# vrenkens/tfkaldi

Hardware: AMD Instinct MI355X
Metric: acoustic frames/sec (train step) (higher is better)
Workload: dtype f32 emulated (3xbf16 planes, 6 products, f32 accumulate)

## Files before the change

tfkaldi_amd/csrc/gemm_bf16.hip:

```cpp
#include "gemm_bf16.h"
#include "x3_layout.h"

#include <math.h>
#include <stdlib.h>
#include <string.h>

#include <type_traits>

namespace tfk {
namespace {

typedef __bf16 bf16x8 __attribute__((ext_vector_type(8)));
typedef __bf16 bf16x4 __attribute__((ext_vector_type(4)));
typedef float f32x16 __attribute__((ext_vector_type(16)));
typedef uint32_t u32x4 __attribute__((ext_vector_type(4)));
typedef int i32x4 __attribute__((ext_vector_type(4)));

constexpr int BK = 64;
constexpr int kOOB = (int)0x80000000;
constexpr int NUM_XCD = 8;

__device__ __forceinline__ void tile_of_seq(int tiles_m, int tiles_n, int group_rows, int seq, int& tm, int& tn) {
  const int per_group = group_rows * tiles_n;
  const int grp = seq / per_group;
// ... 324 lines not shown
  template <bool GUARD>
  __device__ __forceinline__ void issue(int j, unsigned image, int k0, int wave) const {
    const int off = (!GUARD || k0 + kidx[j] < k_lim) ? voff[j] : kOOB;
    const unsigned dst = image + (unsigned)(wave * 64 + j * NTH) * 16u;
    const int soff = k0 * kstride;
    asm volatile("s_mov_b32 m0, %0\n\ts_nop 0\n\tbuffer_load_dwordx4 %1, %2, %3 offen lds"
                 :
                 : "s"(dst), "v"(off), "s"(rsrc), "s"(soff)
                 : "memory");
  }
};

template <bool KC, int EXT, int NF>
struct Frag3 {
  int off[2];
  __device__ __forceinline__ void init(int lane, int frag0) {
#pragma unroll
    for (int v = 0; v < 2; ++v) off[v] = KC ? x3::kc_lane_off(lane, frag0, v) : x3::ks_lane_off<EXT>(lane, frag0, v);
  }
  __device__ __forceinline__ Frag3 at(int bytes) const {
    Frag3 r;
    r.off[0] = off[0] + bytes;
    r.off[1] = off[1] + bytes;
    return r;
  }
  __device__ __forceinline__ bf16x8 read(const char* img, int f, int ks, int pl) const {
    if constexpr (KC) {
      return *reinterpret_cast<const bf16x8*>(img + off[ks] + x3::kc_imm(f, pl));
    } else {
      typedef __attribute__((address_space(3))) bf16x4 lds_bf16x4;
      const int X = 3 * f + pl;
      const char* q = img + off[X & 1];
      const bf16x4 lo = __builtin_amdgcn_ds_read_tr16_b64_v4bf16((lds_bf16x4*)(q + x3::ks_imm<EXT>(X, ks, 0)));
      const bf16x4 hi = __builtin_amdgcn_ds_read_tr16_b64_v4bf16((lds_bf16x4*)(q + x3::ks_imm<EXT>(X, ks, 1)));
      return __builtin_shufflevector(lo, hi, 0, 1, 2, 3, 4, 5, 6, 7);
    }
  }
};

template <bool KC, int EXT, int NF16>
struct Frag3M {
  int off[KC ? 1 : 4];
  __device__ __forceinline__ void init(int lane, int frag0) {
    if constexpr (KC) {
      off[0] = x3::kc16_lane_off(lane, frag0);
    } else {
#pragma unroll
      for (int v = 0; v < 4; ++v) off[v] = x3::ks16_lane_off<EXT>(lane, frag0, v & 1, v >> 1);
    }
  }
  __device__ __forceinline__ Frag3M at(int bytes) const {
    Frag3M r;
#pragma unroll
    for (int v = 0; v < (KC ? 1 : 4); ++v) r.off[v] = off[v] + bytes;
    return r;
  }
  __device__ __forceinline__ bf16x8 read(const char* img, int f, int pl) const {
    if constexpr (KC) {
      return *reinterpret_cast<const bf16x8*>(img + off[0] + x3::kc16_imm(f, pl));
    } else {
      typedef __attribute__((address_space(3))) bf16x4 lds_bf16x4;
      const int X = 3 * (f >> 1) + pl;
      const char* q = img + off[(X & 1) + 2 * (f & 1)];
      const bf16x4 lo = __builtin_amdgcn_ds_read_tr16_b64_v4bf16((lds_bf16x4*)(q + x3::ks16_imm<EXT>(X, 0)));
      const bf16x4 hi = __builtin_amdgcn_ds_read_tr16_b64_v4bf16((lds_bf16x4*)(q + x3::ks16_imm<EXT>(X, 1)));
      return __builtin_shufflevector(lo, hi, 0, 1, 2, 3, 4, 5, 6, 7);
    }
  }
};

#ifndef TFKB_ABL
#define TFKB_ABL 0
#endif

#ifndef TFKB_TL
#define TFKB_TL(ev, ti)
#endif

#define TFKB_WAIT_BARRIER(n) \
  asm volatile("s_waitcnt vmcnt(%0)\n\ts_waitcnt lgkmcnt(0)\n\ts_barrier" : : "n"(n) : "memory")

constexpr int kSplitFlagWords = 4096;
constexpr int kSplitXccWord = 2048;
template <bool A_KC, bool B_KC, int EPI, int WAVES_M, int WAVES_N, int FM, int FN, int NS, int BKT = 64, int SCHED = 0,
          int NPL = 1, int KSPLIT = 1, int LOADERS = 0, bool LIST = false, bool CBUF = false>
__device__ __forceinline__ void dma_tile(const GemmArgsB& p, int tiles_m, int tiles_n, int group_rows, int bid, char* smem,
                                         int seq0 = 0, int ntiles = 1) {
  static_assert(LOADERS == 0 || (NPL == 3 && LOADERS == WAVES_M * WAVES_N), "loader waves: one per multiplying wave, x3 only");
  static_assert(!LIST || (NPL == 3 && KSPLIT == 1 && LOADERS == 0), "tile lists: the unsplit fp32-emulating contraction, no loader waves");
  constexpr int NTH = WAVES_M * WAVES_N * 64;
  constexpr int BM = WAVES_M * FM * 32, BN = WAVES_N * FN * 32;
  typedef typename std::conditional<NPL == 3, DmaOperand3<A_KC, BM, NTH>, DmaOperand<A_KC, BM, NTH, BKT>>::type OA;
  typedef typename std::conditional<NPL == 3, DmaOperand3<B_KC, BN, NTH>, DmaOperand<B_KC, BN, NTH, BKT>>::type OB;
  constexpr int A_BYTES = BM * BKT * 2, B_BYTES = BN * BKT * 2, STAGE = NPL * (A_BYTES + B_BYTES);
  constexpr int NPA = OA::NP, NPB = OB::NP, NP = OA::NP + OB::NP;
  constexpr int KSPT = BKT / 16;
  static_assert(KSPT == 4 || KSPT == 2, "ring slot of 64 or 32 k");
  static_assert(NS >= 3 && (NS - 2) * NP + (NPL == 3 ? NP / 2 : 0) <= 63, "ring depth / vmcnt range");
  static_assert(FM * FN >= 2 || NPL == 3, "two independent accumulator chains per wave");
  static_assert(NPL == 1 || (NPL == 3 && SCHED == 0), "planes");
  static_assert(KSPLIT == 1 || (KSPLIT == 2 && NPL == 3), "split-K: the fp32-emulating contraction only");

  const int tid = threadIdx.x;
  const int lane = tid & 63;
  const int i = lane & 31, h = lane >> 5;
  const int wave = __builtin_amdgcn_readfirstlane(tid >> 6);
  const int wm = wave / WAVES_N, wn = wave % WAVES_N;
  int tm, tn;
  const int khalf = KSPLIT == 2 ? (bid / NUM_XCD) & 1 : 0;
  const int tile_bid = KSPLIT == 2 ? (bid / NUM_XCD >> 1) * NUM_XCD + bid % NUM_XCD : bid;
  if constexpr (LIST) tile_of_seq(tiles_m, tiles_n, group_rows, seq0, tm, tn);
  else tile_of_block(tiles_m, tiles_n, group_rows, tile_bid, tm, tn);
  int m0 = tm * BM, n0 = tn * BN;
  unsigned my_xcc = 0;
  if constexpr (KSPLIT == 2) {
    if (p.splitk_local) {
      asm volatile("s_getreg_b32 %0, hwreg(HW_REG_XCC_ID, 0, 4)" : "=s"(my_xcc));
      if (tid == 0)
        __hip_atomic_store(reinterpret_cast<unsigned*>(p.splitk_ws) + kSplitXccWord + 2 * (tm * tiles_n + tn) + khalf, my_xcc + 1,
                           __ATOMIC_RELAXED, __HIP_MEMORY_SCOPE_AGENT);
    }
  }

  const int K8 = (p.K + 7) & ~7;
  const int nk_all = (p.K + BKT - 1) / BKT;
  const int h0 = KSPLIT == 2 ? max(1, (nk_all + 1) / 2 - p.splitk_skew) : nk_all;
  const int kbase = khalf ? h0 : 0;
  const int nk = KSPLIT == 2 ? (khalf ? nk_all - h0 : h0) : nk_all;
  const int k_end = (kbase + nk) * BKT;
  const unsigned lds0 = __builtin_amdgcn_readfirstlane((unsigned)(unsigned long long)smem);
  OA la;
  OB lb;
  const int a_klim = min(A_KC ? K8 : p.K, k_end), b_klim = min(B_KC ? K8 : p.K, k_end);
  const int nk_full = min(a_klim, b_klim) / BKT - kbase;
  if constexpr (LOADERS > 0) {
    if (wave >= WAVES_M * WAVES_N) {
      const int lwave = wave - WAVES_M * WAVES_N;
      la.init(p.A, p.lda, A_KC ? p.M : p.K, m0, A_KC ? p.M : ((p.M + 7) & ~7), a_klim, tid - NTH);
      lb.init(p.B, p.ldb, B_KC ? p.N : p.K, n0, B_KC ? p.N : ((p.N + 7) & ~7), b_klim, tid - NTH);
      auto tile = [&](auto guard, int slot, int kt) {
        if (TFKB_ABL & 2) return;
#pragma unroll
        for (int j = 0; j < NPA; ++j)
          la.template issue<decltype(guard)::value>(j, lds0 + (unsigned)(slot * STAGE), (kt + kbase) * BKT, lwave);
#pragma unroll
        for (int j = 0; j < NPB; ++j)
          lb.template issue<decltype(guard)::value>(j, lds0 + (unsigned)(slot * STAGE + NPL * A_BYTES), (kt + kbase) * BKT, lwave);
      };
#pragma unroll
      for (int t = 0; t < NS - 1; ++t) tile(std::true_type(), t, t);
      TFKB_WAIT_BARRIER((NS - 2) * NP);
      int ws = NS - 1;
      const int n_fast = max(0, min(nk, nk_full - (NS - 1)));
#pragma unroll 1
      for (int kt = 0; kt < nk; ++kt) {
        if (kt < n_fast) tile(std::false_type(), ws, kt + NS - 1);
        else tile(std::true_type(), ws, kt + NS - 1);
        TFKB_WAIT_BARRIER((NS - 2) * NP);
        ws = ws + 1 == NS ? 0 : ws + 1;
      }
      TFKB_WAIT_BARRIER(0);
      return;
    }
  }
  auto init_loaders = [&]() {
    if constexpr (LOADERS == 0) {
// ... 42 lines not shown
        lb.issue(j - NPA, lds0 + (unsigned)(slot * STAGE + A_BYTES), (kt + kbase) * BKT, wave);
    }
  };
  auto piece = [&](int j, int slot, int kt) { piece_g(std::true_type(), j, slot, kt); };
  constexpr int NPH = NPL == 3 ? NP / 2 : 0;
  auto prologue = [&]() {
#pragma unroll
    for (int t = 0; t < NS - 1; ++t)
#pragma unroll
      for (int j = 0; j < NP; ++j) piece(j, t, t);
#pragma unroll
    for (int j = 0; j < NPH; ++j) piece(j, NS - 1, NS - 1);
    TFKB_WAIT_BARRIER((NS - 2) * NP + NPH);
  };

  bf16x8 fa[2][NPL][FM], fb[2][NPL][FN];
  auto read_frags = [&](int buf, const char* st, int ks) {
    if (TFKB_ABL & 4) return;
#pragma unroll
    for (int pl = 0; pl < NPL; ++pl) {
      if constexpr (NPL == 3) {
#pragma unroll
        for (int a = 0; a < FM; ++a) fa[buf][pl][a] = qa.read(st, a, ks, pl);
#pragma unroll
        for (int b = 0; b < FN; ++b) fb[buf][pl][b] = qb.read(st + NPL * A_BYTES, b, ks, pl);
      } else {
#pragma unroll
        for (int a = 0; a < FM; ++a) fa[buf][pl][a] = qa.read(st, a, ks);
#pragma unroll
        for (int b = 0; b < FN; ++b) fb[buf][pl][b] = qb.read(st + A_BYTES, b, ks);
      }
    }
  };
  if (TFKB_ABL & 4) {
#pragma unroll
    for (int q = 0; q < 2; ++q) {
#pragma unroll
      for (int pl = 0; pl < NPL; ++pl) {
#pragma unroll
        for (int a = 0; a < FM; ++a)
#pragma unroll
          for (int e = 0; e < 8; ++e) fa[q][pl][a][e] = (__bf16)(float)(lane + e + pl);
#pragma unroll
        for (int b = 0; b < FN; ++b)
#pragma unroll
          for (int e = 0; e < 8; ++e) fb[q][pl][b][e] = (__bf16)(float)(lane - e - pl);
      }
    }
  }
  auto mfma_step = [&](int cur) {
    if (TFKB_ABL & 1) {
#pragma unroll
      for (int pl = 0; pl < NPL; ++pl) {
#pragma unroll
        for (int a = 0; a < FM; ++a) asm volatile("" : : "v"(fa[cur][pl][a]));
#pragma unroll
        for (int b = 0; b < FN; ++b) asm volatile("" : : "v"(fb[cur][pl][b]));
      }
    } else if constexpr (NPL == 1) {
#pragma unroll
      for (int a = 0; a < FM; ++a)
#pragma unroll
        for (int b = 0; b < FN; ++b)
          acc[a][b] = __builtin_amdgcn_mfma_f32_32x32x16_bf16(fa[cur][0][a], fb[cur][0][b], acc[a][b], 0, 0, 0);
    } else {
      constexpr int PA[6] = {2, 1, 0, 1, 0, 0}, PB[6] = {0, 1, 2, 0, 1, 0};
#pragma unroll
      for (int c = 0; c < 5; ++c)
#pragma unroll
        for (int a = 0; a < FM; ++a)
#pragma unroll
          for (int b = 0; b < FN; ++b)
            acc2[a][b] = __builtin_amdgcn_mfma_f32_32x32x16_bf16(fa[cur][PA[c]][a], fb[cur][PB[c]][b], acc2[a][b], 0, 0, 0);
#pragma unroll
      for (int a = 0; a < FM; ++a)
#pragma unroll
        for (int b = 0; b < FN; ++b)
          acc[a][b] = __builtin_amdgcn_mfma_f32_32x32x16_bf16(fa[cur][0][a], fb[cur][0][b], acc[a][b], 0, 0, 0);
    }
  };
  constexpr bool CHAIN = LIST && NPL == 3 && TFK_X3_M16 == 0 && SCHED == 0;
  const int nlist = LIST ? ntiles : 1;
  float* const red = reinterpret_cast<float*>(smem + (LIST ? NS * STAGE : 0));
  bool primed = false;
  int rs = 0, ws = NS - 1;
#pragma unroll 1
  for (int ti = 0; ti < nlist; ++ti) {
    TFKB_TL(0, ti);
    if (!primed) {
      if (ti > 0) {
        tile_of_seq(tiles_m, tiles_n, group_rows, seq0 + ti, tm, tn);
        m0 = tm * BM;
        n0 = tn * BN;
        init_loaders();
      }
      prologue();
      rs = 0;
      ws = NS - 1;
    }
    zero_acc();
    const bool chain_next = CHAIN && nk >= NS && ti + 1 < nlist;
    const int tm_out = tm, m0_out = m0, n0_out = n0;
    if constexpr (SCHED == 2) {
      static_assert(WAVES_M * WAVES_N == 8, "two waves per SIMD");
      const int group = wave >> 2;
      bf16x8 wa[KSPT][FM], wb[KSPT][FN];
      if (group == 1) {
        __builtin_amdgcn_sched_barrier(0);
        asm volatile("s_barrier" : : : "memory");
        __builtin_amdgcn_sched_barrier(0);
      }
#pragma unroll 1
      for (int kt = 0; kt < nk; ++kt) {
        const char* st = smem + rs * STAGE;
#pragma unroll
        for (int ks = 0; ks < KSPT; ++ks) {
#pragma unroll
          for (int a = 0; a < FM; ++a) wa[ks][a] = qa.read(st, a, ks);
#pragma unroll
          for (int b = 0; b < FN; ++b) wb[ks][b] = qb.read(st + A_BYTES, b, ks);
        }
#pragma unroll
        for (int j = 0; j < NP; ++j) piece(j, ws, kt + NS - 1);
        __builtin_amdgcn_sched_barrier(0);
        TFKB_WAIT_BARRIER((NS - 2) * NP);
        __builtin_amdgcn_sched_barrier(0);
#pragma unroll
        for (int ks = 0; ks < KSPT; ++ks)
#pragma unroll
          for (int a = 0; a < FM; ++a)
#pragma unroll
            for (int b = 0; b < FN; ++b)
              acc[a][b] = __builtin_amdgcn_mfma_f32_32x32x16_bf16(wa[ks][a], wb[ks][b], acc[a][b], 0, 0, 0);
        rs = rs + 1 == NS ? 0 : rs + 1;
        ws = ws + 1 == NS ? 0 : ws + 1;
        __builtin_amdgcn_sched_barrier(0);
        asm volatile("s_barrier" : : : "memory");
        __builtin_amdgcn_sched_barrier(0);
      }
      if (group == 0) {
        __builtin_amdgcn_sched_barrier(0);
        asm volatile("s_barrier" : : : "memory");
        __builtin_amdgcn_sched_barrier(0);
      }
    } else if constexpr (NPL == 3 && TFK_X3_M16 != 0) {
      static_assert(KSPT == 2, "fp32-emulating contraction: 32 k per ring slot");
      constexpr int FM16 = 2 * FM, FN16 = 2 * FN;
      typedef float f32x4 __attribute__((ext_vector_type(4)));
      Frag3M<A_KC, BM, FM16> ma;
      Frag3M<B_KC, BN, FN16> mb;
      ma.init(lane, wm * FM16);
      mb.init(lane, wn * FN16);
      f32x4 c1[FM16][FN16], c2[FM16][FN16];
#pragma unroll
      for (int a = 0; a < FM16; ++a)
#pragma unroll
        for (int b = 0; b < FN16; ++b) {
          c1[a][b] = f32x4{0.f, 0.f, 0.f, 0.f};
          c2[a][b] = f32x4{0.f, 0.f, 0.f, 0.f};
        }
      bf16x8 ga[3][FM16], gb[3][FN16], gb0n[FN16];
      auto rd_a = [&](const decltype(ma)& r, int pl) {
#pragma unroll
        for (int a = 0; a < FM16; ++a) ga[pl][a] = r.read(smem, a, pl);
      };
      auto rd_b = [&](const decltype(mb)& r, int pl, bf16x8 (&dst)[FN16]) {
#pragma unroll
        for (int b = 0; b < FN16; ++b) dst[b] = r.read(smem, b, pl);
      };
      auto mm = [&](int pa, int pb) {
#pragma unroll
        for (int a = 0; a < FM16; ++a)
#pragma unroll
          for (int b = 0; b < FN16; ++b) {
            if (pa + pb == 0) c1[a][b] = __builtin_amdgcn_mfma_f32_16x16x32_bf16(ga[0][a], gb[0][b], c1[a][b], 0, 0, 0);
            else c2[a][b] = __builtin_amdgcn_mfma_f32_16x16x32_bf16(ga[pa][a], gb[pb][b], c2[a][b], 0, 0, 0);
          }
        __builtin_amdgcn_sched_barrier(0);
      };
      auto pieces = [&](auto guard, int part, int j0, int j1, int slot, int tile) {
#pragma unroll
        for (int j = j0 + part * (j1 - j0) / 3; j < j0 + (part + 1) * (j1 - j0) / 3; ++j) piece_g(guard, j, slot, tile);
      };
      {
        const auto r0a = ma.at(0);
        const auto r0b = mb.at(NPL * A_BYTES);
        rd_a(r0a, 0);
        rd_b(r0b, 0, gb[0]);
        rd_b(r0b, 1, gb[1]);
        rd_b(r0b, 2, gb[2]);
      }
      const int n_fast = max(0, min(nk, nk_full - NS));
      auto iteration = [&](auto guard, int kt) {
        const auto ra = ma.at(rs * STAGE);
        rd_a(ra, 1);
        pieces(guard, 0, NPH, NP, ws, kt + NS - 1);
        mm(0, 0);
        rd_a(ra, 2);
        pieces(guard, 1, NPH, NP, ws, kt + NS - 1);
        mm(0, 1);
        pieces(guard, 2, NPH, NP, ws, kt + NS - 1);
        mm(0, 2);
        TFKB_WAIT_BARRIER((NS - 2) * NP);
        rs = rs + 1 == NS ? 0 : rs + 1;
        ws = ws + 1 == NS ? 0 : ws + 1;
        const bool fetch = kt + 1 < nk;
        const auto na = ma.at(rs * STAGE);
        const auto nb = mb.at(rs * STAGE + NPL * A_BYTES);
        if (fetch) {
          rd_a(na, 0);
          rd_b(nb, 0, gb0n);
        }
        pieces(guard, 0, 0, NPH, ws, kt + NS);
        mm(1, 0);
        if (fetch) rd_b(nb, 2, gb[2]);
        pieces(guard, 1, 0, NPH, ws, kt + NS);
        mm(1, 1);
        if (fetch) rd_b(nb, 1, gb[1]);
        pieces(guard, 2, 0, NPH, ws, kt + NS);
        mm(2, 0);
        if (fetch) {
#pragma unroll
          for (int b = 0; b < FN16; ++b) gb[0][b] = gb0n[b];
        }
      };
#pragma unroll 1
      for (int kt = 0; kt < n_fast; ++kt) iteration(std::false_type(), kt);
#pragma unroll 1
      for (int kt = n_fast; kt < nk; ++kt) iteration(std::true_type(), kt);
      {
        const int src = (16 * h + (i & 15)) * 4;
#pragma unroll
        for (int a = 0; a < FM; ++a)
#pragma unroll
          for (int b = 0; b < FN; ++b)
#pragma unroll
            for (int r = 0; r < 16; ++r) {
              const int addr = src + (((r >> 2) & 1) ? 128 : 0);
              const f32x4& t0 = c1[2 * a + (r >> 3)][2 * b], &u0 = c2[2 * a + (r >> 3)][2 * b];
              const f32x4& t1 = c1[2 * a + (r >> 3)][2 * b + 1], &u1 = c2[2 * a + (r >> 3)][2 * b + 1];
              const float v0 = __builtin_bit_cast(float, __builtin_amdgcn_ds_bpermute(addr, __builtin_bit_cast(int, t0[r & 3] + u0[r & 3])));
              const float v1 = __builtin_bit_cast(float, __builtin_amdgcn_ds_bpermute(addr, __builtin_bit_cast(int, t1[r & 3] + u1[r & 3])));
              acc[a][b][r] = (i & 16) ? v1 : v0;
            }
      }
    } else if constexpr (NPL == 3) {
      static_assert(KSPT == 2, "fp32-emulating contraction: 32 k per ring slot");
      constexpr int PA[6] = {2, 1, 0, 1, 0, 0}, PB[6] = {0, 1, 2, 0, 1, 0};
      auto step3 = [&](auto guard, int cur, bool fetch, const decltype(qa)& ra, const decltype(qb)& rb, int nks, int j0, int j1,
                       int slot, int tile) {
#pragma unroll
        for (int c = 0; c < 6; ++c) {
          if (c < 3 && fetch && !(TFKB_ABL & 4)) {
#pragma unroll
            for (int a = 0; a < FM; ++a) fa[cur ^ 1][PA[c]][a] = ra.read(smem, a, nks, PA[c]);
#pragma unroll
            for (int b = 0; b < FN; ++b) fb[cur ^ 1][PB[c]][b] = rb.read(smem, b, nks, PB[c]);
          }
#pragma unroll
          for (int j = j0 + c * (j1 - j0) / 6; j < j0 + (c + 1) * (j1 - j0) / 6; ++j) piece_g(guard, j, slot, tile);
          if (TFKB_ABL & 1) {
#pragma unroll
            for (int a = 0; a < FM; ++a) asm volatile("" : : "v"(fa[cur][PA[c]][a]));
#pragma unroll
            for (int b = 0; b < FN; ++b) asm volatile("" : : "v"(fb[cur][PB[c]][b]));
          } else {
#pragma unroll
            for (int a = 0; a < FM; ++a)
#pragma unroll
              for (int b = 0; b < FN; ++b) {
                if (c < 5)
                  acc2[a][b] = __builtin_amdgcn_mfma_f32_32x32x16_bf16(fa[cur][PA[c]][a], fb[cur][PB[c]][b], acc2[a][b], 0, 0, 0);
                else
                  acc[a][b] = __builtin_amdgcn_mfma_f32_32x32x16_bf16(fa[cur][PA[c]][a], fb[cur][PB[c]][b], acc[a][b], 0, 0, 0);
              }
          }
          __builtin_amdgcn_sched_barrier(0);
        }
      };
      if (!primed) read_frags(0, smem, 0);
      const int n_fast = max(0, min(nk, nk_full - NS));
      auto iteration = [&](auto guard, int t1, int t2, bool fetch, bool switch_tile) {
        const auto ra = qa.at(rs * STAGE);
        const auto rb = qb.at(rs * STAGE + NPL * A_BYTES);
        step3(guard, 0, true, ra, rb, 1, NPH, NP, ws, t1);
        TFKB_WAIT_BARRIER((NS - 2) * NP);
        rs = rs + 1 == NS ? 0 : rs + 1;
        ws = ws + 1 == NS ? 0 : ws + 1;
        if constexpr (CHAIN) {
          if (switch_tile) {
            tile_of_seq(tiles_m, tiles_n, group_rows, seq0 + ti + 1, tm, tn);
            m0 = tm * BM;
            n0 = tn * BN;
            init_loaders();
          }
        }
        const auto na = qa.at(rs * STAGE);
        const auto nb = qb.at(rs * STAGE + NPL * A_BYTES);
        step3(guard, 1, fetch, na, nb, 0, 0, NPH, ws, t2);
      };
      const int n_own = chain_next ? nk - NS : nk;
      TFKB_TL(1, ti);
#pragma unroll 1
      for (int kt = 0; kt < n_fast; ++kt) iteration(std::false_type(), kt + NS - 1, kt + NS, kt + 1 < nk, false);
#pragma unroll 1
      for (int kt = n_fast; kt < n_own; ++kt) iteration(std::true_type(), kt + NS - 1, kt + NS, kt + 1 < nk, false);
      if constexpr (CHAIN) {
        if (chain_next) {
          iteration(std::true_type(), nk - 1, 0, true, true);
#pragma unroll 1
          for (int t = 0; t < NS - 1; ++t) iteration(std::true_type(), t, t + 1, true, false);
        }
      }
      TFKB_TL(2, ti);
    } else {
    read_frags(0, smem, 0);
#pragma unroll 1
    for (int kt = 0; kt < nk; ++kt) {
      const char* st = smem + rs * STAGE;
#pragma unroll
      for (int ks = 0; ks < KSPT - 1; ++ks) {
        const int cur = ks & 1;
        read_frags(cur ^ 1, st, ks + 1);
#pragma unroll
        for (int j = ks * NP / (KSPT - 1); j < (ks + 1) * NP / (KSPT - 1); ++j) piece(j, ws, kt + NS - 1);
        mfma_step(cur);
        __builtin_amdgcn_sched_barrier(0);
      }
      TFKB_WAIT_BARRIER((NS - 2) * NP);
      rs = rs + 1 == NS ? 0 : rs + 1;
      ws = ws + 1 == NS ? 0 : ws + 1;
      if (kt + 1 < nk) read_frags(0, smem + rs * STAGE, 0);
      mfma_step((KSPT - 1) & 1);
      __builtin_amdgcn_sched_barrier(0);
    }
    }
    if (!chain_next) TFKB_WAIT_BARRIER(0);
    if constexpr (NPL == 3) {
#pragma unroll
      for (int a = 0; a < FM; ++a)
#pragma unroll
        for (int b = 0; b < FN; ++b)
#pragma unroll
          for (int r = 0; r < 16; ++r) acc[a][b][r] += acc2[a][b][r];
    }
    if constexpr (KSPLIT == 2) {
      typedef float f32x4 __attribute__((ext_vector_type(4)));
      unsigned* flags = reinterpret_cast<unsigned*>(p.splitk_ws);
      const int tile = tm * tiles_n + tn;
      constexpr int kSys = 1 | (1 << 4);
      __amdgpu_buffer_rsrc_t part = __builtin_amdgcn_make_buffer_rsrc(
          (void*)(p.splitk_ws + kSplitFlagWords + (size_t)tile * (BM * BN)), 0, BM * BN * 4, 0x00020000);
      unsigned* sh = reinterpret_cast<unsigned*>(smem);
      if (tid == 0) {
        sh[0] = __hip_atomic_fetch_add(&flags[2 * tile], 1u, __ATOMIC_RELAXED, __HIP_MEMORY_SCOPE_AGENT);
        sh[1] = p.splitk_local ? __hip_atomic_load(&flags[kSplitXccWord + 2 * tile + (khalf ^ 1)], __ATOMIC_RELAXED, __HIP_MEMORY_SCOPE_AGENT)
                               : 0u;
      }
      __syncthreads();
      const bool first = sh[0] == 0;
      if (first) {
        const bool same_xcd = p.splitk_local && sh[1] == my_xcc + 1;
        if (same_xcd) {
#pragma unroll
          for (int a = 0; a < FM; ++a)
#pragma unroll
            for (int b = 0; b < FN; ++b)
#pragma unroll
              for (int q = 0; q < 4; ++q)
                __builtin_amdgcn_raw_buffer_store_b128(
                    __builtin_bit_cast(u32x4, f32x4{acc[a][b][4 * q], acc[a][b][4 * q + 1], acc[a][b][4 * q + 2], acc[a][b][4 * q + 3]}),
                    part, ((((wave * FM + a) * FN + b) * 4 + q) * 64 + lane) * 16, 0, 0);
        } else {
#pragma unroll
          for (int a = 0; a < FM; ++a)
#pragma unroll
            for (int b = 0; b < FN; ++b)
#pragma unroll
              for (int q = 0; q < 4; ++q)
                __builtin_amdgcn_raw_buffer_store_b128(
                    __builtin_bit_cast(u32x4, f32x4{acc[a][b][4 * q], acc[a][b][4 * q + 1], acc[a][b][4 * q + 2], acc[a][b][4 * q + 3]}),
                    part, ((((wave * FM + a) * FN + b) * 4 + q) * 64 + lane) * 16, 0, kSys);
        }
        asm volatile("s_waitcnt vmcnt(0)" : : : "memory");
        __syncthreads();
        if (tid == 0) __hip_atomic_store(&flags[2 * tile + 1], 1u, __ATOMIC_RELAXED, __HIP_MEMORY_SCOPE_AGENT);
        return;
      }
      if (tid == 0) {
        int spin = 0;
        for (; spin < (1 << 23) && __hip_atomic_load(&flags[2 * tile + 1], __ATOMIC_RELAXED, __HIP_MEMORY_SCOPE_AGENT) == 0; ++spin)
          __builtin_amdgcn_s_sleep(2);
        if (spin == (1 << 23) && p.err) __hip_atomic_store(p.err, 1u, __ATOMIC_RELAXED, __HIP_MEMORY_SCOPE_SYSTEM);
        __hip_atomic_store(&flags[2 * tile], 0u, __ATOMIC_RELAXED, __HIP_MEMORY_SCOPE_AGENT);
        __hip_atomic_store(&flags[2 * tile + 1], 0u, __ATOMIC_RELAXED, __HIP_MEMORY_SCOPE_AGENT);
        __hip_atomic_store(&flags[kSplitXccWord + 2 * tile], 0u, __ATOMIC_RELAXED, __HIP_MEMORY_SCOPE_AGENT);
        __hip_atomic_store(&flags[kSplitXccWord + 2 * tile + 1], 0u, __ATOMIC_RELAXED, __HIP_MEMORY_SCOPE_AGENT);
      }
      __syncthreads();
#pragma unroll
      for (int a = 0; a < FM; ++a)
#pragma unroll
        for (int b = 0; b < FN; ++b)
#pragma unroll
          for (int q = 0; q < 4; ++q) {
            const f32x4 o = __builtin_bit_cast(
                f32x4, __builtin_amdgcn_raw_buffer_load_b128(part, ((((wave * FM + a) * FN + b) * 4 + q) * 64 + lane) * 16, 0, kSys));
            acc[a][b][4 * q] += o.x;
            acc[a][b][4 * q + 1] += o.y;
            acc[a][b][4 * q + 2] += o.z;
            acc[a][b][4 * q + 3] += o.w;
          }
      __syncthreads();
    }
    epilogue<EPI, WAVES_M, WAVES_N, FM, FN, CBUF>(p, acc, tiles_m, tm_out, m0_out, n0_out, wm, wn, i, h, red);
    TFKB_TL(3, ti);
    if constexpr (LIST) {
      primed = chain_next;
      if (!chain_next && ti + 1 < nlist) __syncthreads();
    }
  }
}

template <bool A_KC, bool B_KC, int EPI, int WAVES_M, int WAVES_N, int FM, int FN, int NS, int BKT = 64, int SCHED = 0,
          int NPL = 1, int KSPLIT = 1, int LOADERS = 0>
__global__ void __launch_bounds__((WAVES_M * WAVES_N + LOADERS) * 64)
gemm_bf16_dma_kernel(GemmArgsB p, int tiles_m, int tiles_n, int group_rows) {
  extern __shared__ __attribute__((aligned(16))) char smem[];
  dma_tile<A_KC, B_KC, EPI, WAVES_M, WAVES_N, FM, FN, NS, BKT, SCHED, NPL, KSPLIT, LOADERS>(p, tiles_m, tiles_n, group_rows,
                                                                                            blockIdx.x, smem);
}

template <int EPI_NT, int EPI_TN, int GWM, int GWN, int GFM, int GFN, int GNS, int HWM, int HWN, int HFM, int HFN, int HNS,
          int HBK>
__global__ void __launch_bounds__(GWM * GWN * 64)
gemm_bf16_dual_kernel(GemmArgsB p1, GemmArgsB p2, int tiles_m1, int tiles_n1, int group1, int tiles_m2, int tiles_n2,
                      int group2) {
  static_assert(GWM * GWN == HWM * HWN, "both halves run on the same block size");
  extern __shared__ __attribute__((aligned(16))) char smem[];
  const int n1 = tiles_m1 * tiles_n1;
  if ((int)blockIdx.x < n1)
    dma_tile<true, true, EPI_NT, GWM, GWN, GFM, GFN, GNS>(p1, tiles_m1, tiles_n1, group1, blockIdx.x, smem);
  else
    dma_tile<false, false, EPI_TN, HWM, HWN, HFM, HFN, HNS, HBK, (HBK == 32 ? 2 : 0)>(p2, tiles_m2, tiles_n2, group2, blockIdx.x - n1,
                                                                                      smem);
}

constexpr int NT = 256, PF = 4;
constexpr int KC_LD = BK + 8;

template <bool KC, int EXT>
struct Operand {
  static constexpr int LD = KC ? KC_LD : EXT + 32;
  static constexpr int SZ = (KC ? EXT : BK) * LD;
  static constexpr int NCH = EXT * BK / 8 / NT;
};

template <bool KC, int EXT>
struct Loader {
  static constexpr int NCH = Operand<KC, EXT>::NCH;
  __amdgpu_buffer_rsrc_t rsrc;
  int voff[NCH];
  int kidx[NCH];
  int kstride;
  int k_lim;

  static __device__ __forceinline__ void coords(int c, int& r, int& q) {
    if (KC) { r = c >> 3; q = (c & 7) << 3; }
    else { r = c / (EXT / 8); q = (c % (EXT / 8)) << 3; }
  }
  __device__ __forceinline__ void init(const bf16_t* base, int ld, int rows, int ext0, int ext_lim, int k_lim_,
                                       int tid) {
    rsrc = __builtin_amdgcn_make_buffer_rsrc((void*)base, 0, rows * ld * 2, 0x00020000);
    k_lim = k_lim_;
    kstride = KC ? 2 : ld * 2;
#pragma unroll
    for (int j = 0; j < NCH; ++j) {
      int r, q;
      coords(tid + j * NT, r, q);
      if (KC) {
        voff[j] = (ext0 + r < ext_lim) ? ((ext0 + r) * ld + q) * 2 : kOOB;
        kidx[j] = q;
      } else {
        voff[j] = (ext0 + q < ext_lim) ? (r * ld + ext0 + q) * 2 : kOOB;
        kidx[j] = r;
      }
    }
  }
  __device__ __forceinline__ void load(u32x4 (&v)[NCH], int k0) const {
#pragma unroll
    for (int j = 0; j < NCH; ++j) {
      const int off = (k0 + kidx[j] < k_lim) ? voff[j] : kOOB;
      v[j] = __builtin_amdgcn_raw_buffer_load_b128(rsrc, off, k0 * kstride, 0);
    }
  }
  __device__ __forceinline__ void store(const u32x4 (&v)[NCH], bf16_t* s, int tid) const {
#pragma unroll
    for (int j = 0; j < NCH; ++j) {
      int r, q;
      coords(tid + j * NT, r, q);
      *reinterpret_cast<u32x4*>(s + r * Operand<KC, EXT>::LD + q) = v[j];
    }
  }
};

template <bool KC, int LD>
__device__ __forceinline__ bf16x8 fragment(const bf16_t* s, int ext_base, int ks, int lane) {
  if (KC) {
    const int i = lane & 31, kb = lane >> 5;
    return *reinterpret_cast<const bf16x8*>(s + (ext_base + i) * LD + 16 * ks + 8 * kb);
  } else {
    const int kb = lane >> 5, half = (lane >> 4) & 1, j = (lane >> 2) & 3, q = lane & 3;
    const bf16_t* p = s + (16 * ks + 8 * kb + j) * LD + ext_base + 16 * half + 4 * q;
// ... 89 lines not shown
#pragma unroll
          for (int a = 0; a < FM; ++a)
#pragma unroll
            for (int b = 0; b < FN; ++b)
              acc[a][b] = __builtin_amdgcn_mfma_f32_32x32x16_bf16(fa[cur][a], fb[cur][b], acc[a][b], 0, 0, 0);
        }
      }
      __syncthreads();
      bf16_t* t = st0; st0 = st1; st1 = st2; st2 = t;
    }
  }
  if constexpr (ALT) {
#pragma unroll
    for (int r = 0; r < 16; ++r) acc[0][0][r] += acc_alt[r];
  }
  epilogue<EPI, 2, 2, FM, FN>(p, acc, tiles_m, tm, m0, n0, wm, wn, i, h, reinterpret_cast<float*>(smem));
}

template <int EPI_NT, int EPI_TN, int WN>
__global__ void __launch_bounds__(WN == 2 ? 256 : 512)
gemm_bf16x3_dual_kernel(GemmArgsB p1, GemmArgsB p2, int tiles_m1, int tiles_n1, int group1, int tiles_m2, int tiles_n2, int group2,
                        int tn_first, int per) {
  extern __shared__ __attribute__((aligned(16))) char smem[];
  const int n1 = tiles_m1 * tiles_n1, n2 = tiles_m2 * tiles_n2;
  const int b = blockIdx.x;
  constexpr bool LIST = WN != 0;
  constexpr int WNN = WN ? WN : 2, FNN = WN ? 4 / WN : 2, LD = WN ? 0 : 4;
  const int n_long = tn_first ? n2 : n1;
  if (b < n_long) {
    if (tn_first) dma_tile<false, false, EPI_TN, 2, WNN, 2, FNN, 3, 32, 0, 3, 1, LD, false, true>(p2, tiles_m2, tiles_n2, group2, b, smem);
    else dma_tile<true, true, EPI_NT, 2, WNN, 2, FNN, 3, 32, 0, 3, 1, LD, false, true>(p1, tiles_m1, tiles_n1, group1, b, smem);
    return;
  }
  int seq0 = 0, count = 1;
  if constexpr (LIST) {
    x3::dual_block_tiles(tn_first ? n1 : n2, per, b - n_long, seq0, count);
    if (count == 0) return;
  }
  if (tn_first)
    dma_tile<true, true, EPI_NT, 2, WNN, 2, FNN, 3, 32, 0, 3, 1, LD, LIST, true>(p1, tiles_m1, tiles_n1, group1, b - n_long, smem, seq0,
                                                                                 count);
  else
    dma_tile<false, false, EPI_TN, 2, WNN, 2, FNN, 3, 32, 0, 3, 1, LD, LIST, true>(p2, tiles_m2, tiles_n2, group2, b - n_long, smem, seq0,
                                                                                  count);
}

struct CfgB {
  int bm, bn;
};
const CfgB kCfgB[kNumGemmBf16Configs] = {{64, 64}, {128, 64}, {128, 128}, {128, 64}, {128, 128}, {256, 128}, {128, 64}, {256, 128},
                                         {256, 256}};
int g_forced_b = -2;
int g_group_rows = 0;

template <class Kern>
int launch_grid(Kern kern, const GemmArgsB& p, int bm, int bn, int threads, size_t lds, hipStream_t stream, bool* attr_done,
                int blocks_per_tile = 1) {
  const int tiles_m = (p.M + bm - 1) / bm, tiles_n = (p.N + bn - 1) / bn;
  if (!*attr_done) {
    hipError_t e = hipFuncSetAttribute(reinterpret_cast<const void*>(kern), hipFuncAttributeMaxDynamicSharedMemorySize,
                                       160 * 1024);
    if (e != hipSuccess) return (int)e;
    *attr_done = true;
  }
  int group_rows = g_group_rows;
  if (group_rows <= 0) {
    const double per_xcd = (double)tiles_m * tiles_n / NUM_XCD;
    group_rows = (int)(sqrt(per_xcd * bn / bm) + 0.5);
  }
  if (group_rows < 1) group_rows = 1;
  if (group_rows > tiles_m) group_rows = tiles_m;
  hipLaunchKernelGGL(kern, dim3(tiles_m * tiles_n * blocks_per_tile), dim3(threads), lds, stream, p, tiles_m, tiles_n, group_rows);
  return (int)hipGetLastError();
}

template <bool A_KC, bool B_KC, int EPI, int FM, int FN>
int launch_reg(const GemmArgsB& p, hipStream_t stream) {
  constexpr int BM = 64 * FM, BN = 64 * FN;
  const size_t lds = (size_t)3 * (Operand<A_KC, BM>::SZ + Operand<B_KC, BN>::SZ) * sizeof(bf16_t);
  static bool attr_done = false;
  return launch_grid(&gemm_bf16_kernel<A_KC, B_KC, EPI, FM, FN>, p, BM, BN, NT, lds, stream, &attr_done);
}
template <bool A_KC, bool B_KC, int EPI, int WAVES_M, int WAVES_N, int FM, int FN, int NS, int BKT = 64, int SCHED = 0,
          int NPL = 1, int KSPLIT = 1, int LOADERS = 0>
int launch_dma(const GemmArgsB& p, hipStream_t stream) {
  constexpr int BM = WAVES_M * FM * 32, BN = WAVES_N * FN * 32;
  const size_t lds = (size_t)NS * NPL * (BM + BN) * BKT * 2;
  static_assert((size_t)NS * NPL * (BM + BN) * BKT * 2 <= 160 * 1024, "LDS");
  static bool attr_done = false;
  return launch_grid(&gemm_bf16_dma_kernel<A_KC, B_KC, EPI, WAVES_M, WAVES_N, FM, FN, NS, BKT, SCHED, NPL, KSPLIT, LOADERS>, p,
                     BM, BN, (WAVES_M * WAVES_N + LOADERS) * 64, lds, stream, &attr_done, KSPLIT);
}

int g_x3_cfg = -2;
int x3_cfg() {
  if (g_x3_cfg == -2) {
    const char* q = getenv("TFK_BF16X3_CFG");
    g_x3_cfg = q ? atoi(q) : -1;
  }
  return g_x3_cfg;
}
bool x3_split_shape(bool tn, int M, int N, int K) {
  const long tiles = (long)((M + 127) / 128) * ((N + 127) / 128);
  return !tn && tiles >= 64 && tiles < 200 && tiles % NUM_XCD == 0 && 2 * tiles <= kSplitXccWord && K >= 512;
}
bool x3_split_shape_tn(int M, int N, int K) {
  const long m128 = (M + 127) / 128, tiles128 = m128 * ((N + 127) / 128), tiles64 = m128 * ((N + 63) / 64);
  return tiles128 < 100 && tiles64 >= 64 && tiles64 < 200 && tiles64 % NUM_XCD == 0 && 2 * tiles64 <= kSplitXccWord && K >= 512;
}
int x3_waves() {
  static const int w = [] {
    const char* q = getenv("TFK_BF16X3_WAVES");
    const int v = q ? atoi(q) : 8;
    return v == 4 || v == 44 ? v : 8;
  }();
  return w;
}
int x3_handover_local() {
  static const int v = [] {
    const char* q = getenv("TFK_X3_HANDOVER");
    return (q && !strcmp(q, "l2")) ? 1 : 0;
  }();
  return v;
}
int x3_kskew() {
  static const int v = [] {
    const char* q = getenv("TFK_X3_KSKEW");
    const int k = q ? atoi(q) : 1;
    return k < 0 ? 0 : k > 8 ? 8 : k;
  }();
  return v;
}
template <bool A_KC, bool B_KC, int EPI>
int launch_x3(const GemmArgsB& p_in, hipStream_t stream) {
  GemmArgsB p = p_in;
  p.splitk_local = x3_handover_local();
  p.splitk_skew = x3_kskew();
  const int forced = x3_cfg();
  const long m128 = (p.M + 127) / 128, n128 = (p.N + 127) / 128;
  const int wv = x3_waves();
  if constexpr (A_KC) {
    if ((forced == 2 || forced < 0) && p.splitk_ws && x3_split_shape(false, p.M, p.N, p.K) &&
        p.splitk_ws_floats >= (size_t)kSplitFlagWords + (size_t)m128 * n128 * 128 * 128)
      return wv == 8    ? launch_dma<A_KC, B_KC, EPI, 2, 4, 2, 1, 3, 32, 0, 3, 2>(p, stream)
             : wv == 44 ? launch_dma<A_KC, B_KC, EPI, 2, 2, 2, 2, 3, 32, 0, 3, 2, 4>(p, stream)
                        : launch_dma<A_KC, B_KC, EPI, 2, 2, 2, 2, 3, 32, 0, 3, 2>(p, stream);
  } else {
    if ((forced == 3 || (forced < 0 && p.K < 2048)) && m128 * n128 < 100 && (long)((p.M + 63) / 64) * ((p.N + 63) / 64) >= 192)
      return launch_dma<A_KC, B_KC, EPI, 2, 2, 1, 1, 4, 32, 0, 3>(p, stream);
    if ((forced == 2 || forced < 0) && p.splitk_ws && x3_split_shape_tn(p.M, p.N, p.K) &&
        p.splitk_ws_floats >= (size_t)kSplitFlagWords + (size_t)m128 * ((p.N + 63) / 64) * 128 * 64)
      return launch_dma<A_KC, B_KC, EPI, 2, 2, 2, 1, 4, 32, 0, 3, 2>(p, stream);
  }
  const bool big = forced >= 0 ? forced == 1 : m128 * n128 >= 200;
  if (big)
    return wv == 8    ? launch_dma<A_KC, B_KC, EPI, 2, 4, 2, 1, 3, 32, 0, 3>(p, stream)
           : wv == 44 ? launch_dma<A_KC, B_KC, EPI, 2, 2, 2, 2, 3, 32, 0, 3, 1, 4>(p, stream)
                      : launch_dma<A_KC, B_KC, EPI, 2, 2, 2, 2, 3, 32, 0, 3>(p, stream);
  return launch_dma<A_KC, B_KC, EPI, 2, 2, 2, 1, 4, 32, 0, 3>(p, stream);
}

template <bool A_KC, bool B_KC, int EPI>
int launch(const GemmArgsB& p, hipStream_t stream) {
  int cfg = gemm_bf16_pick_config(p.M, p.N);
  if constexpr (!A_KC && !B_KC) {
    if (cfg == 8 || (g_forced_b < 0 && (long)((p.M + 255) / 256) * ((p.N + 255) / 256) >= 200))
      return launch_dma<false, false, EPI, 4, 2, 2, 4, 4, 32, 2>(p, stream);
  }
  if (cfg == 8) cfg = 5;
  switch (cfg) {
    case 0: return launch_reg<A_KC, B_KC, EPI, 1, 1>(p, stream);
    case 1: return launch_reg<A_KC, B_KC, EPI, 2, 1>(p, stream);
    case 2: return launch_reg<A_KC, B_KC, EPI, 2, 2>(p, stream);
    case 3: return launch_dma<A_KC, B_KC, EPI, 2, 2, 2, 1, 5>(p, stream);
    case 4: return launch_dma<A_KC, B_KC, EPI, 2, 2, 2, 2, 4>(p, stream);
    case 5: return launch_dma<A_KC, B_KC, EPI, 4, 2, 2, 2, 3>(p, stream);
    case 6: return launch_dma<A_KC, B_KC, EPI, 2, 2, 2, 1, 3>(p, stream);
    case 7: return launch_dma<A_KC, B_KC, EPI, 2, 2, 4, 2, 3>(p, stream);
  }
  return (int)hipErrorInvalidValue;
}

int pick_group_rows(int tiles_m, int tiles_n, int bm, int bn) {
  int group_rows = g_group_rows;
  if (group_rows <= 0) {
    const double per_xcd = (double)tiles_m * tiles_n / NUM_XCD;
    group_rows = (int)(sqrt(per_xcd * bn / bm) + 0.5);
  }
  if (group_rows < 1) group_rows = 1;
  if (group_rows > tiles_m) group_rows = tiles_m;
  return group_rows;
}

template <int EPI_NT, int EPI_TN, int GWM, int GWN, int GFM, int GFN, int GNS, int HWM, int HWN, int HFM, int HFN, int HNS, int HBK>
int launch_dual(const GemmArgsB& a, const GemmArgsB& w, hipStream_t stream) {
  constexpr int BMA = GWM * GFM * 32, BNA = GWN * GFN * 32, BMW = HWM * HFM * 32, BNW = HWN * HFN * 32;
  constexpr size_t lds_a = (size_t)GNS * (BMA + BNA) * 128, lds_w = (size_t)HNS * (BMW + BNW) * HBK * 2;
  constexpr size_t lds = lds_a > lds_w ? lds_a : lds_w;
  static_assert(lds <= 160 * 1024, "LDS");
  auto kern = &gemm_bf16_dual_kernel<EPI_NT, EPI_TN, GWM, GWN, GFM, GFN, GNS, HWM, HWN, HFM, HFN, HNS, HBK>;
  static bool attr_done = false;
  if (!attr_done) {
    hipError_t e = hipFuncSetAttribute(reinterpret_cast<const void*>(kern), hipFuncAttributeMaxDynamicSharedMemorySize,
                                       160 * 1024);
    if (e != hipSuccess) return (int)e;
    attr_done = true;
  }
  const int tma = (a.M + BMA - 1) / BMA, tna = (a.N + BNA - 1) / BNA, tmw = (w.M + BMW - 1) / BMW, tnw = (w.N + BNW - 1) / BNW;
  hipLaunchKernelGGL(kern, dim3(tma * tna + tmw * tnw), dim3(GWM * GWN * 64), lds, stream, a, w, tma, tna,
                     pick_group_rows(tma, tna, BMA, BNA), tmw, tnw, pick_group_rows(tmw, tnw, BMW, BNW));
  return (int)hipGetLastError();
}

template <int GWM, int GWN, int GFM, int GFN, int GNS, int HWM, int HWN, int HFM, int HFN, int HNS, int HBK>
int launch_dual_epi(const GemmArgsB& a, const GemmArgsB& w, hipStream_t stream) {
  const int key = (a.epi == EPI_DACT ? 2 : 0) + (w.epi == EPI_ACCUM ? 1 : 0);
  switch (key) {
    case 0: return launch_dual<0, 0, GWM, GWN, GFM, GFN, GNS, HWM, HWN, HFM, HFN, HNS, HBK>(a, w, stream);
    case 1: return launch_dual<0, EPI_ACCUM, GWM, GWN, GFM, GFN, GNS, HWM, HWN, HFM, HFN, HNS, HBK>(a, w, stream);
    case 2: return launch_dual<EPI_DACT, 0, GWM, GWN, GFM, GFN, GNS, HWM, HWN, HFM, HFN, HNS, HBK>(a, w, stream);
    default: return launch_dual<EPI_DACT, EPI_ACCUM, GWM, GWN, GFM, GFN, GNS, HWM, HWN, HFM, HFN, HNS, HBK>(a, w, stream);
  }
}

int g_dual_cfg = -2;

}

int gemm_bf16_dual_config(int M_nt, int N_nt, int M_tn, int N_tn) {
  if (g_dual_cfg == -2) {
    const char* q = getenv("TFK_BF16_DUAL_CFG");
    g_dual_cfg = q ? atoi(q) : -1;
  }
  if (g_dual_cfg == 0) return 0;
  if (g_dual_cfg == 3 || g_dual_cfg == 4 || g_dual_cfg == 5 || g_dual_cfg == 8) return g_dual_cfg;
  auto tiles = [](int M, int N, int bm, int bn) { return (long)((M + bm - 1) / bm) * ((N + bn - 1) / bn); };
  if (tiles(M_nt, N_nt, 256, 128) >= 200 && tiles(M_tn, N_tn, 256, 256) >= 200) return 8;
  if (tiles(M_nt, N_nt, 256, 128) + tiles(M_tn, N_tn, 256, 128) >= 512) return 5;
  if (tiles(M_nt, N_nt, 128, 128) + tiles(M_tn, N_tn, 128, 128) >= 256) return 4;
  if (tiles(M_nt, N_nt, 128, 64) + tiles(M_tn, N_tn, 128, 64) >= 256) return 3;
  return 0;
}
// ... 147 lines not shown
```

Baseline: 963,800.

## Take split-K ticket early and route x3 launches through CBUF epilogue form

Moves the split-K ticket atomic (and partner XCC load) from after the main loop into the middle of the K loop. The result is stashed in a small extra LDS area past the ring, so the atomic latency and one __syncthreads before the reduction are hidden. It also adds a launch_x3_form wrapper that picks the CBUF epilogue variant for non-activation epilogues when the output fits a 31-bit byte range. That changes how most x3 configs write results. Risks include a ticket taken earlier with respect to the partner's progress and a slightly larger LDS footprint.

```diff
diff --git a/tfkaldi_amd/csrc/gemm_bf16.hip b/tfkaldi_amd/csrc/gemm_bf16.hip
--- a/tfkaldi_amd/csrc/gemm_bf16.hip
+++ b/tfkaldi_amd/csrc/gemm_bf16.hip
@@ -430,6 +430,7 @@
 
 constexpr int kSplitFlagWords = 4096;
 constexpr int kSplitXccWord = 2048;
+constexpr int kSplitTicketBytes = 16;
 template <bool A_KC, bool B_KC, int EPI, int WAVES_M, int WAVES_N, int FM, int FN, int NS, int BKT = 64, int SCHED = 0,
           int NPL = 1, int KSPLIT = 1, int LOADERS = 0, bool LIST = false, bool CBUF = false>
 __device__ __forceinline__ void dma_tile(const GemmArgsB& p, int tiles_m, int tiles_n, int group_rows, int bid, char* smem,
@@ -638,6 +639,20 @@
   constexpr bool CHAIN = LIST && NPL == 3 && TFK_X3_M16 == 0 && SCHED == 0;
   const int nlist = LIST ? ntiles : 1;
   float* const red = reinterpret_cast<float*>(smem + (LIST ? NS * STAGE : 0));
+  unsigned* const flags = reinterpret_cast<unsigned*>(p.splitk_ws);
+  const int split_tile = tm * tiles_n + tn;
+  unsigned ticket, partner_xcc;
+  auto take_ticket = [&]() {
+    if constexpr (KSPLIT == 2) {
+      if (tid == 0) {
+        unsigned word = 2u * (unsigned)split_tile;
+        asm volatile("" : "+v"(word));
+        ticket = __hip_atomic_fetch_add(&flags[word], 1u, __ATOMIC_RELAXED, __HIP_MEMORY_SCOPE_AGENT);
+        if (p.splitk_local)
+          partner_xcc = __hip_atomic_load(&flags[kSplitXccWord + (word | (unsigned)(khalf ^ 1))], __ATOMIC_RELAXED, __HIP_MEMORY_SCOPE_AGENT);
+      }
+    }
+  };
   bool primed = false;
   int rs = 0, ws = NS - 1;
 #pragma unroll 1
@@ -782,6 +797,7 @@
       };
 #pragma unroll 1
       for (int kt = 0; kt < n_fast; ++kt) iteration(std::false_type(), kt);
+      take_ticket();
 #pragma unroll 1
       for (int kt = n_fast; kt < nk; ++kt) iteration(std::true_type(), kt);
       {
@@ -859,6 +875,7 @@
       TFKB_TL(1, ti);
 #pragma unroll 1
       for (int kt = 0; kt < n_fast; ++kt) iteration(std::false_type(), kt + NS - 1, kt + NS, kt + 1 < nk, false);
+      take_ticket();
 #pragma unroll 1
       for (int kt = n_fast; kt < n_own; ++kt) iteration(std::true_type(), kt + NS - 1, kt + NS, kt + 1 < nk, false);
       if constexpr (CHAIN) {
@@ -891,6 +908,13 @@
       __builtin_amdgcn_sched_barrier(0);
     }
     }
+    unsigned* const sh = reinterpret_cast<unsigned*>(smem + NS * STAGE);
+    if constexpr (KSPLIT == 2) {
+      if (tid == 0) {
+        sh[0] = ticket;
+        if (p.splitk_local) sh[1] = partner_xcc;
+      }
+    }
     if (!chain_next) TFKB_WAIT_BARRIER(0);
     if constexpr (NPL == 3) {
 #pragma unroll
@@ -902,19 +926,12 @@
     }
     if constexpr (KSPLIT == 2) {
       typedef float f32x4 __attribute__((ext_vector_type(4)));
-      unsigned* flags = reinterpret_cast<unsigned*>(p.splitk_ws);
-      const int tile = tm * tiles_n + tn;
+      const int tile = split_tile;
       constexpr int kSys = 1 | (1 << 4);
       __amdgpu_buffer_rsrc_t part = __builtin_amdgcn_make_buffer_rsrc(
           (void*)(p.splitk_ws + kSplitFlagWords + (size_t)tile * (BM * BN)), 0, BM * BN * 4, 0x00020000);
-      unsigned* sh = reinterpret_cast<unsigned*>(smem);
-      if (tid == 0) {
-        sh[0] = __hip_atomic_fetch_add(&flags[2 * tile], 1u, __ATOMIC_RELAXED, __HIP_MEMORY_SCOPE_AGENT);
-        sh[1] = p.splitk_local ? __hip_atomic_load(&flags[kSplitXccWord + 2 * tile + (khalf ^ 1)], __ATOMIC_RELAXED, __HIP_MEMORY_SCOPE_AGENT)
-                               : 0u;
-      }
-      __syncthreads();
       const bool first = sh[0] == 0;
+      TFKB_TL(4, ti);
       if (first) {
         const bool same_xcd = p.splitk_local && sh[1] == my_xcc + 1;
         if (same_xcd) {
@@ -941,12 +958,14 @@
         asm volatile("s_waitcnt vmcnt(0)" : : : "memory");
         __syncthreads();
         if (tid == 0) __hip_atomic_store(&flags[2 * tile + 1], 1u, __ATOMIC_RELAXED, __HIP_MEMORY_SCOPE_AGENT);
+        TFKB_TL(5, ti);
         return;
       }
       if (tid == 0) {
         int spin = 0;
         for (; spin < (1 << 23) && __hip_atomic_load(&flags[2 * tile + 1], __ATOMIC_RELAXED, __HIP_MEMORY_SCOPE_AGENT) == 0; ++spin)
           __builtin_amdgcn_s_sleep(2);
+        TFKB_TL(6, ti);
         if (spin == (1 << 23) && p.err) __hip_atomic_store(p.err, 1u, __ATOMIC_RELAXED, __HIP_MEMORY_SCOPE_SYSTEM);
         __hip_atomic_store(&flags[2 * tile], 0u, __ATOMIC_RELAXED, __HIP_MEMORY_SCOPE_AGENT);
         __hip_atomic_store(&flags[2 * tile + 1], 0u, __ATOMIC_RELAXED, __HIP_MEMORY_SCOPE_AGENT);
@@ -968,6 +987,7 @@
             acc[a][b][4 * q + 3] += o.w;
           }
       __syncthreads();
+      TFKB_TL(7, ti);
     }
     epilogue<EPI, WAVES_M, WAVES_N, FM, FN, CBUF>(p, acc, tiles_m, tm_out, m0_out, n0_out, wm, wn, i, h, red);
     TFKB_TL(3, ti);
@@ -979,12 +999,12 @@
 }
 
 template <bool A_KC, bool B_KC, int EPI, int WAVES_M, int WAVES_N, int FM, int FN, int NS, int BKT = 64, int SCHED = 0,
-          int NPL = 1, int KSPLIT = 1, int LOADERS = 0>
+          int NPL = 1, int KSPLIT = 1, int LOADERS = 0, bool CBUF = false>
 __global__ void __launch_bounds__((WAVES_M * WAVES_N + LOADERS) * 64)
 gemm_bf16_dma_kernel(GemmArgsB p, int tiles_m, int tiles_n, int group_rows) {
   extern __shared__ __attribute__((aligned(16))) char smem[];
-  dma_tile<A_KC, B_KC, EPI, WAVES_M, WAVES_N, FM, FN, NS, BKT, SCHED, NPL, KSPLIT, LOADERS>(p, tiles_m, tiles_n, group_rows,
-                                                                                            blockIdx.x, smem);
+  dma_tile<A_KC, B_KC, EPI, WAVES_M, WAVES_N, FM, FN, NS, BKT, SCHED, NPL, KSPLIT, LOADERS, false, CBUF>(
+      p, tiles_m, tiles_n, group_rows, blockIdx.x, smem);
 }
 
 template <int EPI_NT, int EPI_TN, int GWM, int GWN, int GFM, int GFN, int GNS, int HWM, int HWN, int HFM, int HFN, int HNS,
@@ -1240,14 +1260,22 @@
   return launch_grid(&gemm_bf16_kernel<A_KC, B_KC, EPI, FM, FN>, p, BM, BN, NT, lds, stream, &attr_done);
 }
 template <bool A_KC, bool B_KC, int EPI, int WAVES_M, int WAVES_N, int FM, int FN, int NS, int BKT = 64, int SCHED = 0,
-          int NPL = 1, int KSPLIT = 1, int LOADERS = 0>
+          int NPL = 1, int KSPLIT = 1, int LOADERS = 0, bool CBUF = false>
 int launch_dma(const GemmArgsB& p, hipStream_t stream) {
   constexpr int BM = WAVES_M * FM * 32, BN = WAVES_N * FN * 32;
-  const size_t lds = (size_t)NS * NPL * (BM + BN) * BKT * 2;
-  static_assert((size_t)NS * NPL * (BM + BN) * BKT * 2 <= 160 * 1024, "LDS");
+  constexpr size_t lds = (size_t)NS * NPL * (BM + BN) * BKT * 2 + (KSPLIT == 2 ? kSplitTicketBytes : 0);
+  static_assert(lds <= 160 * 1024, "LDS");
   static bool attr_done = false;
-  return launch_grid(&gemm_bf16_dma_kernel<A_KC, B_KC, EPI, WAVES_M, WAVES_N, FM, FN, NS, BKT, SCHED, NPL, KSPLIT, LOADERS>, p,
+  return launch_grid(&gemm_bf16_dma_kernel<A_KC, B_KC, EPI, WAVES_M, WAVES_N, FM, FN, NS, BKT, SCHED, NPL, KSPLIT, LOADERS, CBUF>, p,
                      BM, BN, (WAVES_M * WAVES_N + LOADERS) * 64, lds, stream, &attr_done, KSPLIT);
+}
+template <bool A_KC, bool B_KC, int EPI, int WAVES_M, int WAVES_N, int FM, int FN, int NS, int KSPLIT>
+int launch_x3_form(const GemmArgsB& p, hipStream_t stream) {
+  if constexpr ((EPI & EPI_EVAL_ACT) == 0) {
+    if ((long)p.M * p.ldc * 4 < (1L << 31))
+      return launch_dma<A_KC, B_KC, EPI, WAVES_M, WAVES_N, FM, FN, NS, 32, 0, 3, KSPLIT, 0, true>(p, stream);
+  }
+  return launch_dma<A_KC, B_KC, EPI, WAVES_M, WAVES_N, FM, FN, NS, 32, 0, 3, KSPLIT, 0, false>(p, stream);
 }
 
 int g_x3_cfg = -2;
@@ -1300,22 +1328,22 @@
   if constexpr (A_KC) {
     if ((forced == 2 || forced < 0) && p.splitk_ws && x3_split_shape(false, p.M, p.N, p.K) &&
         p.splitk_ws_floats >= (size_t)kSplitFlagWords + (size_t)m128 * n128 * 128 * 128)
-      return wv == 8    ? launch_dma<A_KC, B_KC, EPI, 2, 4, 2, 1, 3, 32, 0, 3, 2>(p, stream)
+      return wv == 8    ? launch_x3_form<A_KC, B_KC, EPI, 2, 4, 2, 1, 3, 2>(p, stream)
              : wv == 44 ? launch_dma<A_KC, B_KC, EPI, 2, 2, 2, 2, 3, 32, 0, 3, 2, 4>(p, stream)
                         : launch_dma<A_KC, B_KC, EPI, 2, 2, 2, 2, 3, 32, 0, 3, 2>(p, stream);
   } else {
     if ((forced == 3 || (forced < 0 && p.K < 2048)) && m128 * n128 < 100 && (long)((p.M + 63) / 64) * ((p.N + 63) / 64) >= 192)
-      return launch_dma<A_KC, B_KC, EPI, 2, 2, 1, 1, 4, 32, 0, 3>(p, stream);
+      return launch_x3_form<A_KC, B_KC, EPI, 2, 2, 1, 1, 4, 1>(p, stream);
     if ((forced == 2 || forced < 0) && p.splitk_ws && x3_split_shape_tn(p.M, p.N, p.K) &&
         p.splitk_ws_floats >= (size_t)kSplitFlagWords + (size_t)m128 * ((p.N + 63) / 64) * 128 * 64)
-      return launch_dma<A_KC, B_KC, EPI, 2, 2, 2, 1, 4, 32, 0, 3, 2>(p, stream);
+      return launch_x3_form<A_KC, B_KC, EPI, 2, 2, 2, 1, 4, 2>(p, stream);
   }
   const bool big = forced >= 0 ? forced == 1 : m128 * n128 >= 200;
   if (big)
-    return wv == 8    ? launch_dma<A_KC, B_KC, EPI, 2, 4, 2, 1, 3, 32, 0, 3>(p, stream)
+    return wv == 8    ? launch_x3_form<A_KC, B_KC, EPI, 2, 4, 2, 1, 3, 1>(p, stream)
            : wv == 44 ? launch_dma<A_KC, B_KC, EPI, 2, 2, 2, 2, 3, 32, 0, 3, 1, 4>(p, stream)
                       : launch_dma<A_KC, B_KC, EPI, 2, 2, 2, 2, 3, 32, 0, 3>(p, stream);
-  return launch_dma<A_KC, B_KC, EPI, 2, 2, 2, 1, 4, 32, 0, 3>(p, stream);
+  return launch_x3_form<A_KC, B_KC, EPI, 2, 2, 2, 1, 4, 1>(p, stream);
 }
 
 template <bool A_KC, bool B_KC, int EPI>
```

Measured after the change: 972,900, median of 6. No clear change (+0.9%).
